# IXarea/LittleGAN

Hardware: AMD Instinct MI355X
Metric: 128x128 CelebA-shaped images/sec (G+D+Adj step) (higher is better)
Workload: dtype bf16; 1 GPU; C3: 128x128x3 synthetic CelebA, batch 256/GPU, bf16 MFMA conv/transposed-conv + Adjuster branch; global_batch=256, per_gpu_batch=256, image=128, cond_dim=40, parallelism=dp1, launch=eager launches

## Files before the change

### littlegan_amd/csrc/wgrad_at.hip

```cpp
#include "lg_internal.h"

#ifndef LG_WGAT_DBG
#define LG_WGAT_DBG 0
#endif

namespace {

struct WgAtParams {
  const __bf16* big;
  const __bf16* small;
  float* slab;
  int B, Hm, Wm, Cb, Cs;
  int nuj, nunits;
  int items_total, items_per;
};

template <int SW, int R>
struct AtCfg {
  static constexpr bool PAIR = SW == 8;
  static_assert(PAIR ? R == 8 : R * SW / 16 == 8, "8 k steps per item");
  static constexpr int NS = PAIR ? 2 : 1;
  static constexpr int NA = SW + 2;
  static constexpr int EVEN_OFF = NA * 64;
  static constexpr int ROWP = 2 * NA * 64;
  static constexpr int NBR = 2 * R + 3, NPX = 2 * SW + 3;
  static constexpr int BIGS = NBR * ROWP;
  static constexpr int BIG = NS * BIGS, SMALL = NS * R * 2 * SW * 64, BUF = BIG + SMALL;
  static constexpr int NBPS = NBR * NPX * 4;
  static constexpr int NBP = NS * NBPS, NBL = (NBP + 511) / 512;
  static constexpr int NSP = NS * R * SW * 8, NSL = NSP / 512;
  static_assert(BUF < 65536, "k-step offsets must fit the ds offset field");
  static_assert(2 * BUF <= 160 * 1024 && 2 * BUF >= 8 * 2 * 4096, "LDS budget; the tap-24 reduction reuses it");
};

__device__ __forceinline__ f32x16 at_mfma(bf16x8 a, bf16x8 b, f32x16 c) {
  if constexpr (LG_WGAT_DBG & 1) { c[0] += (float)a[0] * (float)b[0]; return c; }
  else return __builtin_amdgcn_mfma_f32_32x32x16_bf16(a, b, c, 0, 0, 0);
}
__device__ __forceinline__ bf16x8 rd_tr(const char* p) {
  typedef short s16x8 __attribute__((ext_vector_type(8)));
  const s16x4 lo = __builtin_amdgcn_ds_read_tr16_b64_v4i16((s16x4 __attribute__((address_space(3)))*)(p));
  const s16x4 hi = __builtin_amdgcn_ds_read_tr16_b64_v4i16((s16x4 __attribute__((address_space(3)))*)(p + 256));
  const s16x8 v = {lo[0], lo[1], lo[2], lo[3], hi[0], hi[1], hi[2], hi[3]};
  return __builtin_bit_cast(bf16x8, v);
}

template <int SW, int R>
__global__ __launch_bounds__(512) void wgrad_at_kernel(const WgAtParams p) {
  using C = AtCfg<SW, R>;
  extern __shared__ __attribute__((aligned(16))) char smem[];
  const int tid = threadIdx.x, lane = tid & 63;
  const int wid = __builtin_amdgcn_readfirstlane(tid >> 6);
  const int bx = lg_xcd_remap(blockIdx.x, gridDim.x);
  const int unit = bx % p.nunits, split = bx / p.nunits;
  const int i0 = (unit / p.nuj) * 32, j0 = (unit % p.nuj) * 64;
  const int it0 = split * p.items_per, it1 = min(it0 + p.items_per, p.items_total);
  const int nxs = p.Wm / SW, nyb = p.Hm / R;
  const int Hb = 2 * p.Hm, Wb = 2 * p.Wm;

  u32x4 rbig[C::NBL], rsm[C::NSL];
  auto load_item = [&](int it) {
    int n, yb, xs;
    if constexpr (C::PAIR) { n = 2 * it; yb = 0; xs = 0; }
    else { xs = it % nxs; const int t2 = it / nxs; yb = t2 % nyb; n = t2 / nyb; }
    const int gy0 = 2 * yb * R - 1, gx0 = 2 * xs * SW - 1;
    const __bf16* bbase = p.big + (long long)n * Hb * Wb * p.Cb + i0;
    const __bf16* sbase = p.small + ((long long)(n * p.Hm + yb * R) * p.Wm + xs * SW) * p.Cs + j0;
#pragma unroll
    for (int k = 0; k < C::NBL; ++k) {
      const int q = tid + k * 512, si = C::PAIR ? q / C::NBPS : 0, qs = q - si * C::NBPS;
      const int piece = qs & 3, pp = qs >> 2;
      const int row = pp / C::NPX, px = pp - row * C::NPX;
      const int gy = gy0 + row, gx = gx0 + px;
      u32x4 v = {0u, 0u, 0u, 0u};
      if (q < C::NBP && (unsigned)gy < (unsigned)Hb && (unsigned)gx < (unsigned)Wb)
        v = *reinterpret_cast<const u32x4*>(bbase + ((long long)si * Hb * Wb + (long long)(gy * Wb + gx)) * p.Cb + piece * 8);
      rbig[k] = v;
    }
#pragma unroll
    for (int k = 0; k < C::NSL; ++k) {
      const int q = tid + k * 512, c8 = q & 7, pp = q >> 3;
      if constexpr (C::PAIR) {
        rsm[k] = *reinterpret_cast<const u32x4*>(sbase + (long long)pp * p.Cs + c8 * 8);
      } else {
        const int yy = pp / SW, px = pp % SW;
        rsm[k] = *reinterpret_cast<const u32x4*>(sbase + (long long)(yy * p.Wm + px) * p.Cs + c8 * 8);
      }
    }
  };
  auto store_item = [&](char* buf) {
#pragma unroll
    for (int k = 0; k < C::NBL; ++k) {
      const int q = tid + k * 512, si = C::PAIR ? q / C::NBPS : 0, qs = q - si * C::NBPS;
      const int piece = qs & 3, pp = qs >> 2;
      const int row = pp / C::NPX, px = pp - row * C::NPX;
      if (q < C::NBP)
        *reinterpret_cast<u32x4*>(buf + si * C::BIGS + row * C::ROWP + ((px & 1) ? C::EVEN_OFF : 0) + (px >> 1) * 64 + piece * 16) = rbig[k];
    }
#pragma unroll
    for (int k = 0; k < C::NSL; ++k) {
      const int q = tid + k * 512, c8 = q & 7, pp = q >> 3;
      if constexpr (C::PAIR) {
        const int si = pp >> 6, pix = pp & 63;
        *reinterpret_cast<u32x4*>(buf + C::BIG + ((si * 2 + (c8 >> 2)) * 64 + pix) * 64 + (c8 & 3) * 16) = rsm[k];
      } else {
        const int yy = pp / SW, px = pp % SW;
        *reinterpret_cast<u32x4*>(buf + C::BIG + ((yy * 2 + (c8 >> 2)) * SW + px) * 64 + (c8 & 3) * 16) = rsm[k];
      }
    }
  };

  const int g = lane >> 4, lq = (lane & 15) >> 2, lp = lane & 3;
  const int lanepart = (8 * (g >> 1) + lq) * 64 + (16 * (g & 1) + 4 * lp) * 2;
  const int lanepartA = C::PAIR ? (g >> 1) * 2 * C::ROWP + lq * 64 + (16 * (g & 1) + 4 * lp) * 2 : lanepart;
  int ab[3];
#pragma unroll
  for (int i = 0; i < 3; ++i) {
    const int t = 3 * wid + i, ky = t / 5, kx = t - ky * 5;
    ab[i] = lanepartA + ky * C::ROWP + ((kx & 1) ? C::EVEN_OFF : 0) + (kx >> 1) * 64;
  }
  const int a24 = lanepartA + 4 * C::ROWP + 2 * 64;
  const int bb = lanepart + C::BIG;

  f32x16 acc[3][2], acc24[2];
#pragma unroll
  for (int e = 0; e < 16; ++e) {
#pragma unroll
    for (int i = 0; i < 3; ++i) { acc[i][0][e] = 0.f; acc[i][1][e] = 0.f; }
    acc24[0][e] = 0.f; acc24[1][e] = 0.f;
  }

  if (it0 < it1) {
    load_item(it0);
    store_item(smem);
  }
  __syncthreads();
  for (int it = it0; it < it1; ++it) {
    const int cur = (it - it0) & 1;
    if (it + 1 < it1 && !(LG_WGAT_DBG & 4)) load_item(it + 1);
    const char* sb = smem + cur * C::BUF;
    auto koffA = [](int ks) {
      constexpr int CH = SW / 16 > 0 ? SW / 16 : 1;
      return C::PAIR ? (ks >> 2) * C::BIGS + 4 * (ks & 3) * C::ROWP : 2 * (ks / CH) * C::ROWP + (ks % CH) * 16 * 64;
    };
    auto koffB = [](int ks, int h) {
      constexpr int CH = SW / 16 > 0 ? SW / 16 : 1;
      return C::PAIR ? (((ks >> 2) * 2 + h) * 64 + 16 * (ks & 3)) * 64 : (((ks / CH) * 2 + h) * SW + (ks % CH) * 16) * 64;
    };
    bf16x8 b[2], a0;
#pragma unroll
    for (int h = 0; h < 2; ++h) b[h] = rd_tr(sb + bb + koffB(0, h));
    a0 = rd_tr(sb + ab[0] + koffA(0));
#pragma unroll
    for (int ks = 0; ks < 8; ++ks) {
      __builtin_amdgcn_sched_barrier(0);
      const bf16x8 a1 = (LG_WGAT_DBG & 2) ? a0 : rd_tr(sb + ab[1] + koffA(ks)), a2 = (LG_WGAT_DBG & 2) ? a0 : rd_tr(sb + ab[2] + koffA(ks));
      __builtin_amdgcn_sched_barrier(0);
      acc[0][0] = at_mfma(a0, b[0], acc[0][0]);
      acc[0][1] = at_mfma(a0, b[1], acc[0][1]);
      __builtin_amdgcn_sched_barrier(0);
      bf16x8 bn[2] = {b[0], b[1]}, a0n = a0;
      if (ks + 1 < 8 && !(LG_WGAT_DBG & 2)) {
#pragma unroll
        for (int h = 0; h < 2; ++h) bn[h] = rd_tr(sb + bb + koffB(ks + 1, h));
        a0n = rd_tr(sb + ab[0] + koffA(ks + 1));
      }
      __builtin_amdgcn_sched_barrier(0);
      acc[1][0] = at_mfma(a1, b[0], acc[1][0]);
      acc[1][1] = at_mfma(a1, b[1], acc[1][1]);
      acc[2][0] = at_mfma(a2, b[0], acc[2][0]);
      acc[2][1] = at_mfma(a2, b[1], acc[2][1]);
      if (wid == ks) {
        const bf16x8 a3 = rd_tr(sb + a24 + koffA(ks));
#pragma unroll
        for (int h = 0; h < 2; ++h) acc24[h] = at_mfma(a3, b[h], acc24[h]);
      }
      b[0] = bn[0]; b[1] = bn[1]; a0 = a0n;
    }
    if (it + 1 < it1 && !(LG_WGAT_DBG & 4)) store_item(smem + (cur ^ 1) * C::BUF);
    __syncthreads();
  }

  const int r = lane & 31, hh = lane >> 5;
  float* out = p.slab + (long long)split * 25 * p.Cb * p.Cs;
#pragma unroll
  for (int i = 0; i < 3; ++i) {
    float* o = out + (long long)(3 * wid + i) * p.Cb * p.Cs + (long long)i0 * p.Cs + j0;
#pragma unroll
    for (int h = 0; h < 2; ++h)
#pragma unroll
      for (int e = 0; e < 16; ++e) o[(long long)((e & 3) + 8 * (e >> 2) + 4 * hh) * p.Cs + h * 32 + r] = acc[i][h][e];
  }
  float* sred = reinterpret_cast<float*>(smem);
#pragma unroll
  for (int h = 0; h < 2; ++h)
#pragma unroll
    for (int e = 0; e < 16; ++e) sred[((wid * 2 + h) * 16 + e) * 64 + lane] = acc24[h][e];
  __syncthreads();
  {
    const int h = tid >> 8, e4 = (tid >> 6) & 3;
    float* o = out + (long long)24 * p.Cb * p.Cs + (long long)i0 * p.Cs + j0;
#pragma unroll
    for (int q = 0; q < 4; ++q) {
      float s = 0.f;
#pragma unroll
      for (int w = 0; w < 8; ++w) s += sred[((w * 2 + h) * 16 + 4 * e4 + q) * 64 + lane];
      o[(long long)(q + 8 * e4 + 4 * hh) * p.Cs + h * 32 + r] = s;
    }
  }
}

inline int at_cus() { return lg_device_cus(); }

inline int at_shape(int Hm, int Wm, int cb, int cs) {
  if (cb % 32 || cs % 64 || cb < 32 || cs < 64) return 0;
  if ((cb / 32) * (cs / 64) > 64) return 0;
  if (Wm % 16 == 0 && Hm % 8 == 0) return 16;
  if (Wm % 32 == 0 && Hm % 4 == 0) return 32;
  if (Wm == 8 && Hm == 8) return 8;
  return 0;
}

inline void at_plan(int B, int Hm, int Wm, int cb, int cs, int sw, int* nsplit, int* items_total, int* items_per) {
  const int R = sw == 32 ? 4 : 8;
  const int nunits = (cb / 32) * (cs / 64);
  *items_total = sw == 8 ? B / 2 : B * (Hm / R) * (Wm / sw);
  int ns = at_cus() / nunits;
  if (ns < 1) ns = 1;
  if (ns > *items_total) ns = *items_total;
  *items_per = lg_cdiv(*items_total, ns);
  *nsplit = lg_cdiv(*items_total, *items_per);
}

}

extern "C" size_t lg_wgrad_at_workspace_bytes(int B, int Hm, int Wm, int cb, int cs) {
  const int sw = at_shape(Hm, Wm, cb, cs);
  if (!sw || (sw == 8 && (B & 1))) return 0;
  int ns, tot, per;
  at_plan(B, Hm, Wm, cb, cs, sw, &ns, &tot, &per);
  return (size_t)ns * 25 * cb * cs * sizeof(float);
}

extern "C" int lg_wgrad_at_try(const void* big16, const void* small16, void* workspace, size_t ws_bytes, int B, int Hm, int Wm,
                               int cb, int cs, int* nsplit_out, void* stream) {
  static int off = -1;
  if (off < 0) off = lg_env_flag("LG_NO_WGAT") ? 1 : 0;
  const int sw = at_shape(Hm, Wm, cb, cs);
  if (off || !sw || (sw == 8 && (B & 1)) || !big16 || !small16 || !nsplit_out) return LG_ERR_UNSUPPORTED;
  WgAtParams p{};
  p.big = (const __bf16*)big16; p.small = (const __bf16*)small16; p.slab = (float*)workspace;
  p.B = B; p.Hm = Hm; p.Wm = Wm; p.Cb = cb; p.Cs = cs;
  p.nuj = cs / 64; p.nunits = (cb / 32) * (cs / 64);
  int ns;
  at_plan(B, Hm, Wm, cb, cs, sw, &ns, &p.items_total, &p.items_per);
  LG_CHECK_ARG(ws_bytes >= (size_t)ns * 25 * cb * cs * sizeof(float), "lg_wgrad_at: workspace too small");
  hipStream_t st = (hipStream_t)stream;
  static bool attr = false;
  if (!attr) {
    (void)hipFuncSetAttribute(reinterpret_cast<const void*>(wgrad_at_kernel<32, 4>), hipFuncAttributeMaxDynamicSharedMemorySize, 2 * AtCfg<32, 4>::BUF);
    (void)hipFuncSetAttribute(reinterpret_cast<const void*>(wgrad_at_kernel<16, 8>), hipFuncAttributeMaxDynamicSharedMemorySize, 2 * AtCfg<16, 8>::BUF);
    (void)hipFuncSetAttribute(reinterpret_cast<const void*>(wgrad_at_kernel<8, 8>), hipFuncAttributeMaxDynamicSharedMemorySize, 2 * AtCfg<8, 8>::BUF);
    attr = true;
  }
  constexpr int LDS32 = 2 * AtCfg<32, 4>::BUF, LDS16 = 2 * AtCfg<16, 8>::BUF, LDS8 = 2 * AtCfg<8, 8>::BUF;
  if (sw == 32) hipLaunchKernelGGL((wgrad_at_kernel<32, 4>), dim3(p.nunits * ns), dim3(512), LDS32, st, p);
  else if (sw == 16) hipLaunchKernelGGL((wgrad_at_kernel<16, 8>), dim3(p.nunits * ns), dim3(512), LDS16, st, p);
  else hipLaunchKernelGGL((wgrad_at_kernel<8, 8>), dim3(p.nunits * ns), dim3(512), LDS8, st, p);
  LG_CHECK_LAUNCH("lg_wgrad_at");
  lg_note_kernel(sw == 32 ? "wgrad_at_kernel<32,4>" : sw == 16 ? "wgrad_at_kernel<16,8>" : "wgrad_at_kernel<8,8>");
  *nsplit_out = ns;
  return LG_OK;
}
```

Baseline: 23560 images/sec.

## Interleave next-item global loads and LDS stores into the MFMA loop via buffer loads

Replaces the bulk load_item/store_item prefetch with per-k-step staging: each of the 8 k steps commits one previously loaded piece to the other LDS buffer and issues one new buffer_load, spreading memory traffic across the MFMA stream. Loads now use raw buffer resources with precomputed per-thread offsets, and border handling goes through a packed edge bitmask with out-of-range offsets, so the per-item index math and branches go away. The wave-specific 25th tap MFMA is moved out of the divergent in-loop branch to the end of the item. It also adds a guard rejecting shapes whose spans would overflow 32-bit buffer offsets. The cost is more live registers and a more complex two-item-deep prefetch schedule.

```diff
diff --git a/littlegan_amd/csrc/wgrad_at.hip b/littlegan_amd/csrc/wgrad_at.hip
--- a/littlegan_amd/csrc/wgrad_at.hip
+++ b/littlegan_amd/csrc/wgrad_at.hip
@@ -1,4 +1,5 @@
 #include "lg_internal.h"
+#include <type_traits>
 
 #ifndef LG_WGAT_DBG
 #define LG_WGAT_DBG 0
@@ -58,56 +59,67 @@
   const int nxs = p.Wm / SW, nyb = p.Hm / R;
   const int Hb = 2 * p.Hm, Wb = 2 * p.Wm;
 
-  u32x4 rbig[C::NBL], rsm[C::NSL];
-  auto load_item = [&](int it) {
-    int n, yb, xs;
-    if constexpr (C::PAIR) { n = 2 * it; yb = 0; xs = 0; }
-    else { xs = it % nxs; const int t2 = it / nxs; yb = t2 % nyb; n = t2 / nyb; }
-    const int gy0 = 2 * yb * R - 1, gx0 = 2 * xs * SW - 1;
-    const __bf16* bbase = p.big + (long long)n * Hb * Wb * p.Cb + i0;
-    const __bf16* sbase = p.small + ((long long)(n * p.Hm + yb * R) * p.Wm + xs * SW) * p.Cs + j0;
-#pragma unroll
-    for (int k = 0; k < C::NBL; ++k) {
-      const int q = tid + k * 512, si = C::PAIR ? q / C::NBPS : 0, qs = q - si * C::NBPS;
-      const int piece = qs & 3, pp = qs >> 2;
-      const int row = pp / C::NPX, px = pp - row * C::NPX;
-      const int gy = gy0 + row, gx = gx0 + px;
-      u32x4 v = {0u, 0u, 0u, 0u};
-      if (q < C::NBP && (unsigned)gy < (unsigned)Hb && (unsigned)gx < (unsigned)Wb)
-        v = *reinterpret_cast<const u32x4*>(bbase + ((long long)si * Hb * Wb + (long long)(gy * Wb + gx)) * p.Cb + piece * 8);
-      rbig[k] = v;
-    }
-#pragma unroll
-    for (int k = 0; k < C::NSL; ++k) {
-      const int q = tid + k * 512, c8 = q & 7, pp = q >> 3;
-      if constexpr (C::PAIR) {
-        rsm[k] = *reinterpret_cast<const u32x4*>(sbase + (long long)pp * p.Cs + c8 * 8);
-      } else {
-        const int yy = pp / SW, px = pp % SW;
-        rsm[k] = *reinterpret_cast<const u32x4*>(sbase + (long long)(yy * p.Wm + px) * p.Cs + c8 * 8);
-      }
-    }
-  };
-  auto store_item = [&](char* buf) {
-#pragma unroll
-    for (int k = 0; k < C::NBL; ++k) {
-      const int q = tid + k * 512, si = C::PAIR ? q / C::NBPS : 0, qs = q - si * C::NBPS;
-      const int piece = qs & 3, pp = qs >> 2;
-      const int row = pp / C::NPX, px = pp - row * C::NPX;
-      if (q < C::NBP)
-        *reinterpret_cast<u32x4*>(buf + si * C::BIGS + row * C::ROWP + ((px & 1) ? C::EVEN_OFF : 0) + (px >> 1) * 64 + piece * 16) = rbig[k];
-    }
-#pragma unroll
-    for (int k = 0; k < C::NSL; ++k) {
-      const int q = tid + k * 512, c8 = q & 7, pp = q >> 3;
-      if constexpr (C::PAIR) {
-        const int si = pp >> 6, pix = pp & 63;
-        *reinterpret_cast<u32x4*>(buf + C::BIG + ((si * 2 + (c8 >> 2)) * 64 + pix) * 64 + (c8 & 3) * 16) = rsm[k];
-      } else {
-        const int yy = pp / SW, px = pp % SW;
-        *reinterpret_cast<u32x4*>(buf + C::BIG + ((yy * 2 + (c8 >> 2)) * SW + px) * 64 + (c8 & 3) * 16) = rsm[k];
-      }
-    }
+  constexpr int NPC = C::NBL + C::NSL;
+  static_assert(NPC == 8, "one staged piece per k step");
+  static_assert(C::NBL * 5 <= 32, "border bits of the big pieces share one register");
+  constexpr unsigned OOB = 0x80000000u;
+  unsigned goff[NPC];
+  int loff[NPC];
+  unsigned bmask = 0;
+#pragma unroll
+  for (int k = 0; k < C::NBL; ++k) {
+    const int q = tid + k * 512, si = C::PAIR ? q / C::NBPS : 0, qs = q - si * C::NBPS;
+    const int piece = qs & 3, pp = qs >> 2;
+    const int row = pp / C::NPX, px = pp - row * C::NPX;
+    goff[k] = (unsigned)((((si * Hb + row) * Wb + px) * p.Cb + piece * 8) * 2);
+    loff[k] = si * C::BIGS + row * C::ROWP + ((px & 1) ? C::EVEN_OFF : 0) + (px >> 1) * 64 + piece * 16;
+    const unsigned m = (row == 0 ? 1u : 0u) | (row >= C::NBR - 2 ? 2u : 0u) | (px == 0 ? 4u : 0u) | (px >= C::NPX - 2 ? 8u : 0u) |
+                       (q >= C::NBP ? 16u : 0u);
+    bmask |= m << (5 * k);
+  }
+#pragma unroll
+  for (int k = 0; k < C::NSL; ++k) {
+    const int q = tid + k * 512, c8 = q & 7, pp = q >> 3;
+    if constexpr (C::PAIR) {
+      const int si = pp >> 6, pix = pp & 63;
+      goff[C::NBL + k] = (unsigned)((pp * p.Cs + c8 * 8) * 2);
+      loff[C::NBL + k] = C::BIG + ((si * 2 + (c8 >> 2)) * 64 + pix) * 64 + (c8 & 3) * 16;
+    } else {
+      const int yy = pp / SW, px = pp % SW;
+      goff[C::NBL + k] = (unsigned)(((yy * p.Wm + px) * p.Cs + c8 * 8) * 2);
+      loff[C::NBL + k] = C::BIG + ((yy * 2 + (c8 >> 2)) * SW + px) * 64 + (c8 & 3) * 16;
+    }
+  }
+  const bool mine_last = tid < C::NBP - (C::NBL - 1) * 512;
+
+  int ci = it0, cxs = 0, cyb = 0, cn = 2 * it0;
+  if constexpr (!C::PAIR) { cxs = it0 % nxs; const int t2 = it0 / nxs; cyb = t2 % nyb; cn = t2 / nyb; }
+  const int big_bytes = (C::NS * Hb * Wb * p.Cb - i0) * 2, small_bytes = (C::NS * p.Hm * p.Wm * p.Cs - j0) * 2;
+  __amdgpu_buffer_rsrc_t rsb, rss;
+  int obig = 0, osm = 0;
+  unsigned edge = 0;
+  auto next_item = [&]() {
+    const int nrec_b = ci < it1 ? big_bytes : 0, nrec_s = ci < it1 ? small_bytes : 0;
+    rsb = __builtin_amdgcn_make_buffer_rsrc(const_cast<__bf16*>(p.big + (long long)cn * Hb * Wb * p.Cb + i0), 0, nrec_b, 0x00027000);
+    rss = __builtin_amdgcn_make_buffer_rsrc(const_cast<__bf16*>(p.small + (long long)cn * p.Hm * p.Wm * p.Cs + j0), 0, nrec_s, 0x00027000);
+    obig = (((2 * cyb * R - 1) * Wb + 2 * cxs * SW - 1) * p.Cb) * 2;
+    osm = ((cyb * R * p.Wm + cxs * SW) * p.Cs) * 2;
+    const unsigned e = (cyb == 0 ? 1u : 0u) | (cyb == nyb - 1 ? 2u : 0u) | (cxs == 0 ? 4u : 0u) | (cxs == nxs - 1 ? 8u : 0u) | 16u;
+    edge = e * 0x02108421u;
+    ++ci;
+    if constexpr (C::PAIR) cn += 2;
+    else if (++cxs == nxs) { cxs = 0; if (++cyb == nyb) { cyb = 0; ++cn; } }
+  };
+  u32x4 rp[NPC];
+  auto request = [&](int k) {
+    unsigned off;
+    if (k < C::NBL) off = (bmask & (edge & (0x1fu << (5 * k)))) ? OOB : goff[k] + (unsigned)obig;
+    else off = goff[k] + (unsigned)osm;
+    if (k < C::NBL) rp[k] = __builtin_bit_cast(u32x4, __builtin_amdgcn_raw_buffer_load_b128(rsb, off, 0, 0));
+    else rp[k] = __builtin_bit_cast(u32x4, __builtin_amdgcn_raw_buffer_load_b128(rss, off, 0, 0));
+  };
+  auto commit = [&](int k, char* buf) {
+    if (k != C::NBL - 1 || mine_last) *reinterpret_cast<u32x4*>(buf + loff[k]) = rp[k];
   };
 
   const int g = lane >> 4, lq = (lane & 15) >> 2, lp = lane & 3;
@@ -119,8 +131,17 @@
     const int t = 3 * wid + i, ky = t / 5, kx = t - ky * 5;
     ab[i] = lanepartA + ky * C::ROWP + ((kx & 1) ? C::EVEN_OFF : 0) + (kx >> 1) * 64;
   }
-  const int a24 = lanepartA + 4 * C::ROWP + 2 * 64;
   const int bb = lanepart + C::BIG;
+  auto koffA = [](int ks) {
+    constexpr int CH = SW / 16 > 0 ? SW / 16 : 1;
+    return C::PAIR ? (ks >> 2) * C::BIGS + 4 * (ks & 3) * C::ROWP : 2 * (ks / CH) * C::ROWP + (ks % CH) * 16 * 64;
+  };
+  auto koffB = [](int ks, int h) {
+    constexpr int CH = SW / 16 > 0 ? SW / 16 : 1;
+    return C::PAIR ? (((ks >> 2) * 2 + h) * 64 + 16 * (ks & 3)) * 64 : (((ks / CH) * 2 + h) * SW + (ks % CH) * 16) * 64;
+  };
+  const int a24 = lanepartA + 4 * C::ROWP + 2 * 64 + koffA(wid);
+  const int b24[2] = {bb + koffB(wid, 0), bb + koffB(wid, 1)};
 
   f32x16 acc[3][2], acc24[2];
 #pragma unroll
@@ -130,23 +151,8 @@
     acc24[0][e] = 0.f; acc24[1][e] = 0.f;
   }
 
-  if (it0 < it1) {
-    load_item(it0);
-    store_item(smem);
-  }
-  __syncthreads();
-  for (int it = it0; it < it1; ++it) {
-    const int cur = (it - it0) & 1;
-    if (it + 1 < it1 && !(LG_WGAT_DBG & 4)) load_item(it + 1);
-    const char* sb = smem + cur * C::BUF;
-    auto koffA = [](int ks) {
-      constexpr int CH = SW / 16 > 0 ? SW / 16 : 1;
-      return C::PAIR ? (ks >> 2) * C::BIGS + 4 * (ks & 3) * C::ROWP : 2 * (ks / CH) * C::ROWP + (ks % CH) * 16 * 64;
-    };
-    auto koffB = [](int ks, int h) {
-      constexpr int CH = SW / 16 > 0 ? SW / 16 : 1;
-      return C::PAIR ? (((ks >> 2) * 2 + h) * 64 + 16 * (ks & 3)) * 64 : (((ks / CH) * 2 + h) * SW + (ks % CH) * 16) * 64;
-    };
+  auto run_item = [&](auto stage_c, const char* sb, char* wb) {
+    constexpr bool STAGE = decltype(stage_c)::value && !(LG_WGAT_DBG & 4);
     bf16x8 b[2], a0;
 #pragma unroll
     for (int h = 0; h < 2; ++h) b[h] = rd_tr(sb + bb + koffB(0, h));
@@ -160,24 +166,50 @@
       acc[0][1] = at_mfma(a0, b[1], acc[0][1]);
       __builtin_amdgcn_sched_barrier(0);
       bf16x8 bn[2] = {b[0], b[1]}, a0n = a0;
-      if (ks + 1 < 8 && !(LG_WGAT_DBG & 2)) {
-#pragma unroll
-        for (int h = 0; h < 2; ++h) bn[h] = rd_tr(sb + bb + koffB(ks + 1, h));
-        a0n = rd_tr(sb + ab[0] + koffA(ks + 1));
+      if (!(LG_WGAT_DBG & 2)) {
+        if (ks + 1 < 8) {
+#pragma unroll
+          for (int h = 0; h < 2; ++h) bn[h] = rd_tr(sb + bb + koffB(ks + 1, h));
+          a0n = rd_tr(sb + ab[0] + koffA(ks + 1));
+        } else {
+#pragma unroll
+          for (int h = 0; h < 2; ++h) bn[h] = rd_tr(sb + b24[h]);
+          a0n = rd_tr(sb + a24);
+        }
       }
+      if constexpr (STAGE) { commit(ks, wb); request(ks); }
       __builtin_amdgcn_sched_barrier(0);
       acc[1][0] = at_mfma(a1, b[0], acc[1][0]);
       acc[1][1] = at_mfma(a1, b[1], acc[1][1]);
       acc[2][0] = at_mfma(a2, b[0], acc[2][0]);
       acc[2][1] = at_mfma(a2, b[1], acc[2][1]);
-      if (wid == ks) {
-        const bf16x8 a3 = rd_tr(sb + a24 + koffA(ks));
-#pragma unroll
-        for (int h = 0; h < 2; ++h) acc24[h] = at_mfma(a3, b[h], acc24[h]);
-      }
       b[0] = bn[0]; b[1] = bn[1]; a0 = a0n;
     }
-    if (it + 1 < it1 && !(LG_WGAT_DBG & 4)) store_item(smem + (cur ^ 1) * C::BUF);
+    __builtin_amdgcn_sched_barrier(0);
+#pragma unroll
+    for (int h = 0; h < 2; ++h) acc24[h] = at_mfma(a0, b[h], acc24[h]);
+  };
+
+  if (it0 < it1) {
+    next_item();
+#pragma unroll
+    for (int k = 0; k < NPC; ++k) request(k);
+#pragma unroll
+    for (int k = 0; k < NPC; ++k) commit(k, smem);
+    if constexpr (!(LG_WGAT_DBG & 4)) {
+      next_item();
+#pragma unroll
+      for (int k = 0; k < NPC; ++k) request(k);
+    }
+    __syncthreads();
+    int cur = 0;
+    for (int it = it0; it + 1 < it1; ++it) {
+      next_item();
+      run_item(std::true_type{}, smem + cur * C::BUF, smem + (cur ^ 1) * C::BUF);
+      __syncthreads();
+      cur ^= 1;
+    }
+    run_item(std::false_type{}, smem + cur * C::BUF, smem);
     __syncthreads();
   }
 
@@ -248,6 +280,8 @@
   if (off < 0) off = lg_env_flag("LG_NO_WGAT") ? 1 : 0;
   const int sw = at_shape(Hm, Wm, cb, cs);
   if (off || !sw || (sw == 8 && (B & 1)) || !big16 || !small16 || !nsplit_out) return LG_ERR_UNSUPPORTED;
+  const long long span = (sw == 8 ? 2LL : 1LL) * Hm * Wm * 2;
+  if (4 * span * cb >= 0x80000000LL || span * cs >= 0x80000000LL) return LG_ERR_UNSUPPORTED;
   WgAtParams p{};
   p.big = (const __bf16*)big16; p.small = (const __bf16*)small16; p.slab = (float*)workspace;
   p.B = B; p.Hm = Hm; p.Wm = Wm; p.Cb = cb; p.Cs = cs;
```

New measurement: 23790 images/sec, median of 6. No clear change (+1.0%).
